# zhizdev/sparsefusion

Measured on AMD Instinct MI355X. Metric: novel views/sec, distillation steps (2 NGP renders fwd+bwd + VAE enc/dec + 51-eval PLMS + LPIPS), 256^2 / 32x32 latents, 2-view synthetic hydrant, higher is better.
Workload: dtype bf16 MFMA operands / f32 accumulate (UNet); f32 (NGP render)

## Files before the change

### sparsefusion_amd/csrc/ngp_bwd_mfma.h

```cpp
#pragma once
#include "sf_dev.h"
#include "ngp_device.h"

#define FB_PTS 32
#define FB_SF 33
#define FB_SH 65
#define FB_WAVE_FLOATS (FB_PTS * FB_SF + 2 * FB_PTS * FB_SH + FB_PTS * 4 + FB_PTS)
#define FB_W0 0
#define FB_W1 (FB_W0 + NGP_HID * FB_SF)
#define FB_W2 (FB_W1 + NGP_HID * FB_SH)
#define FB_B0 (FB_W2 + NGP_OUT * NGP_HID)
#define FB_B1 (FB_B0 + NGP_HID)
#define FB_B2 (FB_B1 + NGP_HID)
#define FB_WTOT (FB_B2 + 8)
#define FB_LDS_FLOATS (FB_WTOT + 4 * FB_WAVE_FLOATS)

struct FBArgs {
  const float* table; const float* w0; const float* b0; const float* w1; const float* b1; const float* w2; const float* b2;
  float bound;
  long long* g_w0; long long* g_b0; long long* g_w1; long long* g_b1; long long* g_w2; long long* g_b2;
  float* f_w0; float* f_b0; float* f_w1; float* f_b1; float* f_w2; float* f_b2;
  float thr;
  NgpLevels lv;
  const float* rays_o; const float* rays_d; const float* aabb; const float* z_s; const float* dsig; const float* drgb;
  float* dfeat_out;
  uint32_t P, T2;
  uint32_t dfeat_P, p_off;
  const float* feat_c; const float* feat_f; const uint32_t* perm;
};

SF_KERNEL(256) void k_ngp_field_bwd_mfma(FBArgs a) {
  SF_DYN_LDS(lds_raw);
  float* W = reinterpret_cast<float*>(lds_raw);
  const int tid = threadIdx.x, lane = tid & 63, wave = tid >> 6;
  float* F = W + FB_WTOT + wave * FB_WAVE_FLOATS;
  float* H1 = F + FB_PTS * FB_SF;
  float* H2 = H1 + FB_PTS * FB_SH;
  float* DO = H2 + FB_PTS * FB_SH;
  float* INS = DO + FB_PTS * 4;
  for (int i = tid; i < NGP_HID * NGP_FEAT; i += 256) W[FB_W0 + (i >> 5) * FB_SF + (i & 31)] = a.w0[i];
  for (int i = tid; i < NGP_HID * NGP_HID; i += 256) W[FB_W1 + (i >> 6) * FB_SH + (i & 63)] = a.w1[i];
  for (int i = tid; i < NGP_OUT * NGP_HID; i += 256) W[FB_W2 + i] = a.w2[i];
  if (tid < NGP_HID) { W[FB_B0 + tid] = a.b0[tid]; W[FB_B1 + tid] = a.b1[tid]; }
  if (tid < NGP_OUT) W[FB_B2 + tid] = a.b2[tid];
  float box[6];
#pragma unroll
  for (int i = 0; i < 6; ++i) box[i] = a.aabb[i];
  sf_sync();

  const int li = lane & 15, kq = lane >> 4;
  f32x4 acc1[4][4], acc0[4][2];
#pragma unroll
  for (int i = 0; i < 4; ++i) {
#pragma unroll
    for (int j = 0; j < 4; ++j) acc1[i][j] = f32x4{0.f, 0.f, 0.f, 0.f};
    acc0[i][0] = f32x4{0.f, 0.f, 0.f, 0.f};
    acc0[i][1] = f32x4{0.f, 0.f, 0.f, 0.f};
  }
  float acc2[4] = {0.f, 0.f, 0.f, 0.f};
  float accb2 = 0.0f, accb1 = 0.0f, accb0 = 0.0f;

  const uint32_t n_trips = (a.P + FB_PTS - 1) / FB_PTS;
  for (uint32_t trip = blockIdx.x * 4 + wave; trip < n_trips; trip += gridDim.x * 4) {
    const uint32_t p0 = trip * FB_PTS;
    const int pl = lane & 31, half = lane >> 5;
    const uint32_t p = p0 + pl;
    const bool live = p < a.P;
    float x[3] = {0.f, 0.f, 0.f}, x01[3] = {0.f, 0.f, 0.f};
    bool inside = false;
    if (live) {
      const uint32_t n = p / a.T2;
      const float o[3] = {a.rays_o[n * 3], a.rays_o[n * 3 + 1], a.rays_o[n * 3 + 2]};
      const float d[3] = {a.rays_d[n * 3], a.rays_d[n * 3 + 1], a.rays_d[n * 3 + 2]};
      ngp_point(o, d, a.z_s[p], box, x);
      inside = ngp_unit(x, a.bound, x01);
    }
    if (a.feat_c) {
      f32x4 fv[4];
#pragma unroll
      for (int j = 0; j < 4; ++j) fv[j] = f32x4{0.f, 0.f, 0.f, 0.f};
      if (live) {
        const uint32_t pg = a.p_off + p, n = pg / a.T2, T = a.T2 >> 1;
        const uint32_t src = a.perm[pg];
        const float* row = (src < T ? a.feat_c + ((size_t)n * T + src) * NGP_FEAT : a.feat_f + ((size_t)n * T + (src - T)) * NGP_FEAT) + half * 16;
#pragma unroll
        for (int j = 0; j < 4; ++j) fv[j] = *reinterpret_cast<const f32x4*>(row + 4 * j);
      }
#pragma unroll
      for (int j = 0; j < 4; ++j)
#pragma unroll
        for (int e = 0; e < 4; ++e) F[pl * FB_SF + half * 16 + 4 * j + e] = fv[j][e];
    } else {
#pragma unroll
      for (int ll = 0; ll < 8; ++ll) {
        const uint32_t l = half * 8 + ll;
        float r0 = 0.0f, r1 = 0.0f;
        if (inside && l < a.lv.L) {
          NgpCell c;
          ngp_cell(a.lv, l, x01, c);
          const float* tab = a.table + (size_t)a.lv.offset[l] * 2;
#pragma unroll
          for (int i = 0; i < 8; ++i) {
            const f32x2 fv = *reinterpret_cast<const f32x2*>(tab + (size_t)c.row[i] * 2);
            r0 = fmaf(c.w[i], fv[0], r0);
            r1 = fmaf(c.w[i], fv[1], r1);
          }
        }
        F[pl * FB_SF + 2 * l] = r0;
        F[pl * FB_SF + 2 * l + 1] = r1;
      }
    }
    if (half == 0) INS[pl] = inside ? 1.0f : 0.0f;
    sf_wave_sync();

    {
      f32x4 c[2][4];
#pragma unroll
      for (int nt = 0; nt < 4; ++nt) {
        const float bv = W[FB_B0 + nt * 16 + li];
        c[0][nt] = f32x4{bv, bv, bv, bv};
        c[1][nt] = c[0][nt];
      }
#pragma unroll
      for (int s = 0; s < NGP_FEAT / 4; ++s) {
        const float a0 = F[li * FB_SF + 4 * s + kq], a1 = F[(16 + li) * FB_SF + 4 * s + kq];
#pragma unroll
        for (int nt = 0; nt < 4; ++nt) {
          const float b = W[FB_W0 + (nt * 16 + li) * FB_SF + 4 * s + kq];
          c[0][nt] = sf_mfma4(a0, b, c[0][nt]);
          c[1][nt] = sf_mfma4(a1, b, c[1][nt]);
        }
      }
#pragma unroll
      for (int mt = 0; mt < 2; ++mt)
#pragma unroll
        for (int nt = 0; nt < 4; ++nt)
#pragma unroll
          for (int r = 0; r < 4; ++r) H1[(mt * 16 + 4 * kq + r) * FB_SH + nt * 16 + li] = fmaxf(c[mt][nt][r], 0.0f);
    }
    sf_wave_sync();
    {
      f32x4 c[2][4];
#pragma unroll
      for (int nt = 0; nt < 4; ++nt) {
        const float bv = W[FB_B1 + nt * 16 + li];
        c[0][nt] = f32x4{bv, bv, bv, bv};
        c[1][nt] = c[0][nt];
      }
#pragma unroll
      for (int s = 0; s < NGP_HID / 4; ++s) {
        const float a0 = H1[li * FB_SH + 4 * s + kq], a1 = H1[(16 + li) * FB_SH + 4 * s + kq];
#pragma unroll
        for (int nt = 0; nt < 4; ++nt) {
          const float b = W[FB_W1 + (nt * 16 + li) * FB_SH + 4 * s + kq];
          c[0][nt] = sf_mfma4(a0, b, c[0][nt]);
          c[1][nt] = sf_mfma4(a1, b, c[1][nt]);
        }
      }
#pragma unroll
      for (int mt = 0; mt < 2; ++mt)
#pragma unroll
        for (int nt = 0; nt < 4; ++nt)
#pragma unroll
          for (int r = 0; r < 4; ++r) H2[(mt * 16 + 4 * kq + r) * FB_SH + nt * 16 + li] = fmaxf(c[mt][nt][r], 0.0f);
    }
    sf_wave_sync();
    {
      float o0 = W[FB_B2 + 2 * half], o1 = W[FB_B2 + 2 * half + 1];
#pragma unroll 8
      for (int k = 0; k < NGP_HID; ++k) {
        const float hk = H2[pl * FB_SH + k];
        o0 = fmaf(W[FB_W2 + (2 * half) * NGP_HID + k], hk, o0);
        o1 = fmaf(W[FB_W2 + (2 * half + 1) * NGP_HID + k], hk, o1);
      }
      float d0 = 0.0f, d1 = 0.0f;
      if (live) {
        if (half == 0) {
          const float pre = o0 + ngp_blob(x);
          d0 = a.dsig[p] * expf(fminf(fmaxf(pre, -15.0f), 15.0f));
          const float sg = ngp_sigmoid(o1);
          d1 = a.drgb[p * 3 + 0] * sg * (1.0f - sg);
        } else {
          const float s0 = ngp_sigmoid(o0), s1 = ngp_sigmoid(o1);
          d0 = a.drgb[p * 3 + 1] * s0 * (1.0f - s0);
          d1 = a.drgb[p * 3 + 2] * s1 * (1.0f - s1);
        }
      }
      DO[pl * 4 + 2 * half] = d0;
      DO[pl * 4 + 2 * half + 1] = d1;
    }
    sf_wave_sync();
    {
      float b = 0.0f;
#pragma unroll 4
      for (int q = 0; q < FB_PTS; ++q) {
        const float dv = DO[q * 4 + kq];
#pragma unroll
        for (int i = 0; i < 4; ++i) acc2[i] = fmaf(dv, H2[q * FB_SH + 4 * li + i], acc2[i]);
        b += dv;
      }
      if (li == 0) accb2 += b;
    }
    sf_wave_sync();
    {
      const float w0 = W[FB_W2 + lane], w1 = W[FB_W2 + NGP_HID + lane], w2 = W[FB_W2 + 2 * NGP_HID + lane],
                  w3 = W[FB_W2 + 3 * NGP_HID + lane];
      float b = 0.0f;
#pragma unroll 4
      for (int q = 0; q < FB_PTS; ++q) {
        const f32x4 dv = *reinterpret_cast<const f32x4*>(DO + q * 4);
        const float g = fmaf(w3, dv[3], fmaf(w2, dv[2], fmaf(w1, dv[1], w0 * dv[0])));
        const float m = H2[q * FB_SH + lane] > 0.0f ? g : 0.0f;
        H2[q * FB_SH + lane] = m;
        b += m;
      }
      accb1 += b;
    }
    sf_wave_sync();
#pragma unroll
    for (int s = 0; s < FB_PTS / 4; ++s) {
      float av[4], bv[4];
#pragma unroll
      for (int t = 0; t < 4; ++t) {
        av[t] = H2[(4 * s + kq) * FB_SH + t * 16 + li];
        bv[t] = H1[(4 * s + kq) * FB_SH + t * 16 + li];
      }
#pragma unroll
      for (int jt = 0; jt < 4; ++jt)
#pragma unroll
        for (int kt = 0; kt < 4; ++kt) acc1[jt][kt] = sf_mfma4(av[jt], bv[kt], acc1[jt][kt]);
    }
    {
      f32x4 c[2][4];
#pragma unroll
      for (int nt = 0; nt < 4; ++nt) { c[0][nt] = f32x4{0.f, 0.f, 0.f, 0.f}; c[1][nt] = c[0][nt]; }
#pragma unroll
      for (int s = 0; s < NGP_HID / 4; ++s) {
        const float a0 = H2[li * FB_SH + 4 * s + kq], a1 = H2[(16 + li) * FB_SH + 4 * s + kq];
#pragma unroll
        for (int nt = 0; nt < 4; ++nt) {
          const float b = W[FB_W1 + (4 * s + kq) * FB_SH + nt * 16 + li];
          c[0][nt] = sf_mfma4(a0, b, c[0][nt]);
          c[1][nt] = sf_mfma4(a1, b, c[1][nt]);
        }
      }
      sf_wave_sync();
#pragma unroll
      for (int mt = 0; mt < 2; ++mt)
#pragma unroll
        for (int nt = 0; nt < 4; ++nt)
#pragma unroll
          for (int r = 0; r < 4; ++r) {
            float* hp = H1 + (mt * 16 + 4 * kq + r) * FB_SH + nt * 16 + li;
            *hp = *hp > 0.0f ? c[mt][nt][r] : 0.0f;
          }
    }
    sf_wave_sync();
    {
      float b = 0.0f;
#pragma unroll 8
      for (int q = 0; q < FB_PTS; ++q) b += H1[q * FB_SH + lane];
      accb0 += b;
    }
#pragma unroll
    for (int s = 0; s < FB_PTS / 4; ++s) {
      float av[4], bv[2];
#pragma unroll
      for (int t = 0; t < 4; ++t) av[t] = H1[(4 * s + kq) * FB_SH + t * 16 + li];
      bv[0] = F[(4 * s + kq) * FB_SF + li];
      bv[1] = F[(4 * s + kq) * FB_SF + 16 + li];
#pragma unroll
      for (int jt = 0; jt < 4; ++jt) {
        acc0[jt][0] = sf_mfma4(av[jt], bv[0], acc0[jt][0]);
        acc0[jt][1] = sf_mfma4(av[jt], bv[1], acc0[jt][1]);
      }
    }
    if (a.dfeat_out) {
      f32x4 c[2][2];
      c[0][0] = c[0][1] = c[1][0] = c[1][1] = f32x4{0.f, 0.f, 0.f, 0.f};
#pragma unroll
      for (int s = 0; s < NGP_HID / 4; ++s) {
        const float a0 = H1[li * FB_SH + 4 * s + kq], a1 = H1[(16 + li) * FB_SH + 4 * s + kq];
        const float b0 = W[FB_W0 + (4 * s + kq) * FB_SF + li], b1 = W[FB_W0 + (4 * s + kq) * FB_SF + 16 + li];
        c[0][0] = sf_mfma4(a0, b0, c[0][0]);
        c[0][1] = sf_mfma4(a0, b1, c[0][1]);
        c[1][0] = sf_mfma4(a1, b0, c[1][0]);
        c[1][1] = sf_mfma4(a1, b1, c[1][1]);
      }
      sf_wave_sync();
#pragma unroll
      for (int mt = 0; mt < 2; ++mt)
#pragma unroll
        for (int ft = 0; ft < 2; ++ft)
#pragma unroll
          for (int r = 0; r < 4; ++r) {
            const int q = mt * 16 + 4 * kq + r, f = ft * 16 + li;
            F[q * FB_SF + f] = INS[q] != 0.0f ? c[mt][ft][r] : 0.0f;
          }
      sf_wave_sync();
      {
        const uint32_t l = lane >> 2, q0 = (lane & 3) * 8;
        if (l < a.lv.L) {
          float* dst = a.dfeat_out + ((size_t)l * a.dfeat_P + a.p_off + p0 + q0) * 2;
          if (p0 + FB_PTS <= a.P && !((a.dfeat_P | a.p_off) & 1)) {
#pragma unroll
            for (int j = 0; j < 4; ++j) {
              f32x4 v;
              v[0] = F[(q0 + 2 * j) * FB_SF + 2 * l];     v[1] = F[(q0 + 2 * j) * FB_SF + 2 * l + 1];
              v[2] = F[(q0 + 2 * j + 1) * FB_SF + 2 * l]; v[3] = F[(q0 + 2 * j + 1) * FB_SF + 2 * l + 1];
              *reinterpret_cast<f32x4*>(dst + 4 * j) = v;
            }
          } else {
            for (int j = 0; j < 8; ++j)
              if (p0 + q0 + j < a.P) { dst[2 * j] = F[(q0 + j) * FB_SF + 2 * l]; dst[2 * j + 1] = F[(q0 + j) * FB_SF + 2 * l + 1]; }
          }
        }
      }
    }
    sf_wave_sync();
  }

#pragma unroll
  for (int jt = 0; jt < 4; ++jt)
#pragma unroll
    for (int r = 0; r < 4; ++r) {
      const int j = jt * 16 + 4 * kq + r;
#pragma unroll
      for (int kt = 0; kt < 4; ++kt) sf_grad_add(a.g_w1 + j * NGP_HID + kt * 16 + li, a.f_w1 + j * NGP_HID + kt * 16 + li, acc1[jt][kt][r], a.thr);
      sf_grad_add(a.g_w0 + j * NGP_FEAT + li, a.f_w0 + j * NGP_FEAT + li, acc0[jt][0][r], a.thr);
      sf_grad_add(a.g_w0 + j * NGP_FEAT + 16 + li, a.f_w0 + j * NGP_FEAT + 16 + li, acc0[jt][1][r], a.thr);
    }
#pragma unroll
  for (int i = 0; i < 4; ++i) sf_grad_add(a.g_w2 + kq * NGP_HID + 4 * li + i, a.f_w2 + kq * NGP_HID + 4 * li + i, acc2[i], a.thr);
  if (li == 0) sf_grad_add(a.g_b2 + kq, a.f_b2 + kq, accb2, a.thr);
  sf_grad_add(a.g_b1 + lane, a.f_b1 + lane, accb1, a.thr);
  sf_grad_add(a.g_b0 + lane, a.f_b0 + lane, accb0, a.thr);
}
```

Measured before the change: 18.15.

## Software-prefetch next trip's per-point inputs in NGP field backward kernel

Adds a register-level software pipeline to the NGP field backward MFMA kernel. Each wave loads the ray origin/direction, sample depth, upstream gradients and gathered features for its next trip while it computes the current one. The permutation index is fetched two trips ahead, so the dependent feature gather is not serialized behind it. This is meant to hide global-memory latency in a loop with low occupancy, at the cost of extra live registers that could reduce occupancy or cause spills. Out-of-range points are clamped to the last point so the prefetch stays in bounds.

```diff
diff --git a/sparsefusion_amd/csrc/ngp_bwd_mfma.h b/sparsefusion_amd/csrc/ngp_bwd_mfma.h
--- a/sparsefusion_amd/csrc/ngp_bwd_mfma.h
+++ b/sparsefusion_amd/csrc/ngp_bwd_mfma.h
@@ -28,6 +28,37 @@
   uint32_t dfeat_P, p_off;
   const float* feat_c; const float* feat_f; const uint32_t* perm;
 };
+
+struct FBIn {
+  float z, o[3], d[3];
+  float g0, g1;
+  f32x4 fv[4];
+};
+SF_DEV uint32_t fb_load_perm(const FBArgs& a, uint32_t trip, int lane) {
+  uint32_t p = trip * FB_PTS + (lane & 31);
+  if (p > a.P - 1) p = a.P - 1;
+  return a.feat_c ? a.perm[a.p_off + p] : 0u;
+}
+SF_DEV void fb_load(const FBArgs& a, uint32_t trip, int lane, uint32_t src, FBIn& in) {
+  const int half = lane >> 5;
+  uint32_t p = trip * FB_PTS + (lane & 31);
+  if (p > a.P - 1) p = a.P - 1;
+  const uint32_t n = p / a.T2;
+#pragma unroll
+  for (int i = 0; i < 3; ++i) { in.o[i] = a.rays_o[n * 3 + i]; in.d[i] = a.rays_d[n * 3 + i]; }
+  in.z = a.z_s[p];
+  in.g0 = *(half == 0 ? a.dsig + p : a.drgb + (size_t)p * 3 + 1);
+  in.g1 = a.drgb[(size_t)p * 3 + (half == 0 ? 0 : 2)];
+  if (a.feat_c) {
+    const uint32_t pg = a.p_off + p, ng = pg / a.T2, T = a.T2 >> 1;
+    const float* row = (src < T ? a.feat_c + ((size_t)ng * T + src) * NGP_FEAT : a.feat_f + ((size_t)ng * T + (src - T)) * NGP_FEAT) + half * 16;
+#pragma unroll
+    for (int j = 0; j < 4; ++j) in.fv[j] = *reinterpret_cast<const f32x4*>(row + 4 * j);
+  } else {
+#pragma unroll
+    for (int j = 0; j < 4; ++j) in.fv[j] = f32x4{0.f, 0.f, 0.f, 0.f};
+  }
+}
 
 SF_KERNEL(256) void k_ngp_field_bwd_mfma(FBArgs a) {
   SF_DYN_LDS(lds_raw);
@@ -61,35 +92,41 @@
   float accb2 = 0.0f, accb1 = 0.0f, accb0 = 0.0f;
 
   const uint32_t n_trips = (a.P + FB_PTS - 1) / FB_PTS;
+#ifndef FB_NO_PREFETCH
+  const uint32_t trip0 = blockIdx.x * 4 + wave, trip_step = gridDim.x * 4;
+  FBIn nxt;
+  fb_load(a, trip0, lane, fb_load_perm(a, trip0, lane), nxt);
+  uint32_t src_nn = fb_load_perm(a, trip0 + trip_step, lane);
+  SF_USE_FROM_HERE(nxt.z); SF_USE_FROM_HERE(nxt.g0); SF_USE_FROM_HERE(nxt.g1); SF_USE_FROM_HERE(src_nn);
+#pragma unroll
+  for (int i = 0; i < 3; ++i) { SF_USE_FROM_HERE(nxt.o[i]); SF_USE_FROM_HERE(nxt.d[i]); }
+#pragma unroll
+  for (int j = 0; j < 4; ++j) SF_USE_FROM_HERE(nxt.fv[j]);
+#endif
   for (uint32_t trip = blockIdx.x * 4 + wave; trip < n_trips; trip += gridDim.x * 4) {
     const uint32_t p0 = trip * FB_PTS;
     const int pl = lane & 31, half = lane >> 5;
     const uint32_t p = p0 + pl;
     const bool live = p < a.P;
+#ifdef FB_NO_PREFETCH
+    FBIn in;
+    fb_load(a, trip, lane, fb_load_perm(a, trip, lane), in);
+#else
+    const FBIn in = nxt;
+    fb_load(a, trip + trip_step, lane, src_nn, nxt);
+    src_nn = fb_load_perm(a, trip + 2 * trip_step, lane);
+#endif
     float x[3] = {0.f, 0.f, 0.f}, x01[3] = {0.f, 0.f, 0.f};
     bool inside = false;
     if (live) {
-      const uint32_t n = p / a.T2;
-      const float o[3] = {a.rays_o[n * 3], a.rays_o[n * 3 + 1], a.rays_o[n * 3 + 2]};
-      const float d[3] = {a.rays_d[n * 3], a.rays_d[n * 3 + 1], a.rays_d[n * 3 + 2]};
-      ngp_point(o, d, a.z_s[p], box, x);
+      ngp_point(in.o, in.d, in.z, box, x);
       inside = ngp_unit(x, a.bound, x01);
     }
     if (a.feat_c) {
-      f32x4 fv[4];
-#pragma unroll
-      for (int j = 0; j < 4; ++j) fv[j] = f32x4{0.f, 0.f, 0.f, 0.f};
-      if (live) {
-        const uint32_t pg = a.p_off + p, n = pg / a.T2, T = a.T2 >> 1;
-        const uint32_t src = a.perm[pg];
-        const float* row = (src < T ? a.feat_c + ((size_t)n * T + src) * NGP_FEAT : a.feat_f + ((size_t)n * T + (src - T)) * NGP_FEAT) + half * 16;
-#pragma unroll
-        for (int j = 0; j < 4; ++j) fv[j] = *reinterpret_cast<const f32x4*>(row + 4 * j);
-      }
 #pragma unroll
       for (int j = 0; j < 4; ++j)
 #pragma unroll
-        for (int e = 0; e < 4; ++e) F[pl * FB_SF + half * 16 + 4 * j + e] = fv[j][e];
+        for (int e = 0; e < 4; ++e) F[pl * FB_SF + half * 16 + 4 * j + e] = live ? in.fv[j][e] : 0.0f;
     } else {
 #pragma unroll
       for (int ll = 0; ll < 8; ++ll) {
@@ -177,13 +214,13 @@
       if (live) {
         if (half == 0) {
           const float pre = o0 + ngp_blob(x);
-          d0 = a.dsig[p] * expf(fminf(fmaxf(pre, -15.0f), 15.0f));
+          d0 = in.g0 * expf(fminf(fmaxf(pre, -15.0f), 15.0f));
           const float sg = ngp_sigmoid(o1);
-          d1 = a.drgb[p * 3 + 0] * sg * (1.0f - sg);
+          d1 = in.g1 * sg * (1.0f - sg);
         } else {
           const float s0 = ngp_sigmoid(o0), s1 = ngp_sigmoid(o1);
-          d0 = a.drgb[p * 3 + 1] * s0 * (1.0f - s0);
-          d1 = a.drgb[p * 3 + 2] * s1 * (1.0f - s1);
+          d0 = in.g0 * s0 * (1.0f - s0);
+          d1 = in.g1 * s1 * (1.0f - s1);
         }
       }
       DO[pl * 4 + 2 * half] = d0;
```

New measurement: 18.15 (median of 4 runs). Within noise of the previous version (+0.0%).
